# boguszjelinski/taxidispatcher

Measured on AMD Instinct MI355X. Metric: NxN assignments/sec, higher is better.
Workload: dtype int32; 1 GPU; g1 N=16384: device cost write (4N^2 B) + exact assignment, total checked == optimum; n=16384, parallelism=single GPU

## Files before the change

### taxidispatcher_amd/csrc/td_assign.hip

```cpp
#include <dlfcn.h>
#include <limits.h>
#include <stdlib.h>

#include <type_traits>

#include "td_common.h"

using namespace td;

namespace {

template <typename CT>
struct Tr;
template <>
struct Tr<uint8_t> {
    using PT = int32_t;
    static constexpr int E = 16;
    static constexpr uint32_t SENT = 0xFFu;
    static constexpr int64_t LIMIT = 254;
    static constexpr int32_t BIG = 1 << 28;
    static constexpr int32_t KMAX = INT32_MAX;
};
template <>
struct Tr<uint16_t> {
// ... 124 lines not shown
int g_sapx_min = 8;
int g_sapx_rows = 24;
int g_sap512 = 1;
int g_psap_worth = 4;
int g_bid0 = 1;
int g_defer_const = 1;
int g_shape = 1;
int g_shape_max_n = 1 << 20;
int g_narrow_price = 1;
long long g_np_plimit = NP_PLIMIT;
int g_fuse_t = 2;
int g_fuse_spec = 1;
int g_fused_rounds = 8;
int g_fuse_gen = 1;
int g_tick_rounds = 5;
int g_forest = 1;
int g_forest_min_n = 2048;
long long g_forest_w0 = 16;
long long g_forest_wx = 16;
int g_blocks = -1;
int g_blocks_min_n = 12288;
int g_zs_rounds = 4;
int g_hop_passes = 2;
int g_hop_max_rows = HOP_FMAX;
int g_lazy_cc = 1;
int g_hop_global = 1;
int g_one_trip = 1;
int g_zs_global_rounds = 6;
int g_core = 1;
int g_core_k = 64;
int g_core_min_n = 8192;
int g_core_mode = 1;
double g_core_eps = 1.0;
int g_rand_test = 1;
int g_rand_div = 8192;
int g_rand_rounds = 48;
double g_rand_corr = 0.12;
int g_core_patience = 6;
int g_solver_eps = 0;
int g_eps_theta = 8;
long long g_eps0_mult = 4;
void read_tunables()
{
    static bool done = false;
    if (done) return;
    done = true;
// ... 45 lines not shown
    if (const char *e = getenv("TD_SHAPE_MAX_N")) g_shape_max_n = atoi(e);
    if (const char *e = getenv("TD_WIDE_U16_N")) g_wide_u16_n = std::max(0, atoi(e));
    if (const char *e = getenv("TD_U16_REDO_FREE")) g_u16_redo_free = std::max(0, atoi(e));
    if (const char *e = getenv("TD_WARM_TIE_DIV")) g_warm_tie_div = std::max(1, atoi(e));
    if (const char *e = getenv("TD_LINE")) g_line = atoi(e) != 0;
    if (const char *e = getenv("TD_LINE_MIN_N")) g_line_min_n = std::max(2, atoi(e));
    if (const char *e = getenv("TD_PSAP8_GRID")) g_psap8_grid = std::max(1, std::min(192, atoi(e)));
    if (const char *e = getenv("TD_CORE")) g_core = atoi(e) != 0;
    if (const char *e = getenv("TD_CORE_K")) g_core_k = std::max(2, std::min(200, atoi(e)));
    if (const char *e = getenv("TD_CORE_MIN_N")) g_core_min_n = std::max(256, atoi(e));
    if (const char *e = getenv("TD_CORE_MODE")) g_core_mode = atoi(e);
    if (const char *e = getenv("TD_CORE_EPS")) g_core_eps = atof(e);
    if (const char *e = getenv("TD_CORE_PATIENCE")) g_core_patience = std::max(1, atoi(e));
    if (const char *e = getenv("TD_RAND_TEST")) g_rand_test = atoi(e) != 0;
    if (const char *e = getenv("TD_RAND_DIV")) g_rand_div = std::max(1, atoi(e));
    if (const char *e = getenv("TD_RAND_ROUNDS")) g_rand_rounds = std::max(1, std::min(48, atoi(e)));
    if (const char *e = getenv("TD_RAND_CORR")) g_rand_corr = atof(e);
    if (const char *e = getenv("TD_BLOCKS")) g_blocks = std::max(-1, std::min(HOP_BMAX, atoi(e)));
    if (const char *e = getenv("TD_BLOCKS_MIN_N")) g_blocks_min_n = std::max(0, atoi(e));
    if (const char *e = getenv("TD_ZS_ROUNDS")) g_zs_rounds = std::max(0, std::min(32, atoi(e)));
    if (const char *e = getenv("TD_HOP_PASSES")) g_hop_passes = std::max(0, std::min(8, atoi(e)));
    if (const char *e = getenv("TD_HOP_MAX_ROWS")) g_hop_max_rows = std::max(1, atoi(e));
    if (const char *e = getenv("TD_HOP_GLOBAL")) g_hop_global = atoi(e) != 0;
    if (const char *e = getenv("TD_ONE_TRIP")) g_one_trip = atoi(e) != 0;
    if (const char *e = getenv("TD_LAZY_CC")) g_lazy_cc = atoi(e) != 0;
    if (const char *e = getenv("TD_ZS_GLOBAL_ROUNDS")) g_zs_global_rounds = std::max(1, std::min(48, atoi(e)));
}

template <typename CT>
__device__ __forceinline__ void unpack(const uint4 &v, uint32_t *out);
template <>
__device__ __forceinline__ void unpack<uint8_t>(const uint4 &v, uint32_t *o)
{
    const uint32_t w[4] = {v.x, v.y, v.z, v.w};
#pragma unroll
    for (int k = 0; k < 4; k++) {
        o[4 * k + 0] = w[k] & 0xFFu;
        o[4 * k + 1] = (w[k] >> 8) & 0xFFu;
        o[4 * k + 2] = (w[k] >> 16) & 0xFFu;
        o[4 * k + 3] = w[k] >> 24;
    }
}
template <>
__device__ __forceinline__ void unpack<u8e>(const uint4 &v, uint32_t *o)
{
    const uint32_t w[4] = {v.x, v.y, v.z, v.w};
// ... 735 lines not shown
    for (int o = 1; o < 64; o <<= 1) {
        const int va = __shfl_up(ia, o), vb = __shfl_up(ib, o);
        if (lane >= o) ia += va, ib += vb;
    }
    if (lane == 63) s_fl2_w[0][w] = ia, s_fl2_w[1][w] = ib;
    __syncthreads();
    int basea = 0, baseb = 0;
    for (int k = 0; k < w; k++) basea += s_fl2_w[0][k], baseb += s_fl2_w[1][k];
    if (tid == T - 1) s_fl2_tot[0] = basea + ia, s_fl2_tot[1] = baseb + ib;
    free_list_fill(na, a, lista, wanta, cnta, basea + ia - cnta);
    free_list_fill(nb, b, listb, wantb, cntb, baseb + ib - cntb);
    __syncthreads();
    tota = s_fl2_tot[0], totb = s_fl2_tot[1];
}

__global__ __launch_bounds__(1024) void k_freelist(int n, const int *__restrict__ r2c, int *__restrict__ list,
                                                   int *__restrict__ ctl)
{
    if (ctl[CTL_FLAG]) return;
    const int cnt = build_free_list(n, r2c, list);
    if (threadIdx.x == 0) ctl[CTL_NFREE] = cnt;
}

#include "td_blocks.h"
#include "td_core_warm.h"

__device__ __forceinline__ void place_const_tail(int n, int *__restrict__ r2c, int *__restrict__ owner,
                                                 int *__restrict__ lista, int *__restrict__ listb,
                                                 int *__restrict__ ctl)
{
    if (ctl[CTL_NCONST] == 0) return;
    const int nr = build_free_list(n, r2c, lista, -2);
    if (nr == 0) return;
    const int nc = build_free_list(n, owner, listb, -1);
    if (nc != nr) {
        if (threadIdx.x == 0) atomicOr(&ctl[CTL_ERR], 8);
        return;
    }
    for (int k = threadIdx.x; k < nr; k += blockDim.x) {
        const int r = lista[k], j = listb[k];
        r2c[r] = j;
        owner[j] = r;
    }
}

__global__ __launch_bounds__(1024) void k_place_const(int n, int *__restrict__ r2c, int *__restrict__ owner,
                                                      int *__restrict__ lista, int *__restrict__ listb,
                                                      int *__restrict__ ctl, const int *__restrict__ gate_left = nullptr)
{
    const int flag = __hip_atomic_load(&ctl[CTL_FLAG], __ATOMIC_RELAXED, __HIP_MEMORY_SCOPE_AGENT);
    const int nconst = __hip_atomic_load(&ctl[CTL_NCONST], __ATOMIC_RELAXED, __HIP_MEMORY_SCOPE_AGENT);
    const int left = gate_left ? *gate_left : 0;
    asm volatile("" :: "v"(flag), "v"(nconst), "s"(left));
    if (flag || left != 0 || nconst == 0) return;
    place_const_tail(n, r2c, owner, lista, listb, ctl);
}

__device__ __forceinline__ void shape_decide(int n, int *__restrict__ ctl)
{
    int *sh = ctl + CTL_SHAPE;
    __threadfence();
    const int ncol = atomicAdd(&sh[0], 0);
    const int nrow = atomicAdd(&ctl[CTL_NCONST], 0);
    sh[1] = nrow;
    const int margin = n / 256 > 32 ? n / 256 : 32;
    if (ncol >= 16 && ncol - nrow >= margin) {
        sh[3] = 1;
// ... 1967 lines not shown
    *fits = h[CTL_FLAG] == 0 && *range <= (int64_t)Tr<uint32_t>::LIMIT && *range >= 0;
    sv.nconst = h[CTL_NCONST];
    if (*fits) {
        sv.nchunks = nchunks;
        sv.npad = npad;
    }
    return TD_OK;
}

int sv_complete_cc(Solver &sv)
{
    if (!sv.cc_partial) return TD_OK;
    Ctx &c = ctx();
    ProfScope ps(TD_K_COMPRESS);
    k_compress_rest<<<std::max(1, std::min(sv.nrows, c.n_cu * 8)), 256, 0, c.stream>>>(sv.n, sv.nrows, sv.row0, sv.nchunks, sv.cc_rpb, sv.d_cost,
                                                                                      (uint8_t *)sv.cc.p, (const int32_t *)sv.rowmin.p,
                                                                                      (const int *)sv.misc.p);
    TD_HIP(hipGetLastError());
    sv.cc_partial = false;
    return TD_OK;
}

template <typename CT>
int sv_hop_t(Solver &sv, int rpb, int ncols_blk, int col_lo, int nb, bool window_zero, uint8_t *ob, bool raw = false, bool gate = false)
{
    Ctx &c = ctx();
    using PT = typename Tr<CT>::PT;
    int rc;
    if ((rc = ensure(sv.hop, sizeof(HopCtl)))) return rc;
    if ((rc = ensure(sv.hoptab, sizeof(int) * (size_t)nb * HOP_FMAX * HOP_FMAX))) return rc;
    HopCtl *hc = (HopCtl *)sv.hop.p;
    int *frl = (int *)sv.list.p, *fcl = (int *)sv.pred.p;
    const int *ctl = (const int *)sv.misc.p;
    if (gate && nb != 1) return fail(TD_EINTERNAL, "a gated two-hop pass takes one block");
    const int nseg = raw && window_zero ? (ncols_blk / 4 + 1023) / 1024 : 1;
    k_hop_lists<<<nb, 1024, 0, c.stream>>>(rpb, ncols_blk, col_lo, (const int *)sv.r2c.p, (const int *)sv.owner.p, frl, fcl, hc, ctl,
                                           gate ? g_hop_max_rows : 0, nseg > 1 ? (int *)sv.hoptab.p : nullptr);
    if (raw) {
        if (!sv.d_cost || sv.n % 4) return fail(TD_EINVAL, "two-hop pass on the int32 matrix: no matrix, or n %% 4 != 0");
        if (nseg > 1)
            k_hop_table<CT, true, true><<<nb * HOP_FMAX * nseg, 256, 0, c.stream>>>(
                sv.n, sv.nrows, sv.row0, sv.n / 4, rpb, ncols_blk, col_lo, g_hop_max_rows, 1, (const CT *)sv.d_cost, (const PT *)sv.price.p,
                (const int *)sv.owner.p, frl, fcl, hc, (int *)sv.hoptab.p, ctl, (const int32_t *)sv.rowmin.p, nseg);
        else
        k_hop_table<CT, true><<<nb * HOP_FMAX, 256, 0, c.stream>>>(sv.n, sv.nrows, sv.row0, sv.n / 4, rpb, ncols_blk, col_lo, g_hop_max_rows,
                                                                   window_zero ? 1 : 0, (const CT *)sv.d_cost, (const PT *)sv.price.p,
                                                                   (const int *)sv.owner.p, frl, fcl, hc, (int *)sv.hoptab.p, ctl,
                                                                   (const int32_t *)sv.rowmin.p);
    } else {
    k_hop_table<CT><<<nb * HOP_FMAX, 256, 0, c.stream>>>(sv.n, sv.nrows, sv.row0, sv.nchunks, rpb, ncols_blk, col_lo, g_hop_max_rows,
                                                         window_zero ? 1 : 0, (const CT *)sv.cc.p, (const PT *)sv.price.p,
                                                         (const int *)sv.owner.p, frl, fcl, hc, (int *)sv.hoptab.p, ctl);
    }
    const size_t match_lds = sizeof(uint32_t) * ((size_t)HOP_FMAX * HOP_FMAX + (size_t)((rpb + 31) / 32));
    if (match_lds > 150 * 1024) return fail(TD_EINVAL, "two-hop pass: a block of that many rows does not fit the LDS");
    TD_HIP(hipFuncSetAttribute((const void *)k_hop_match<PT>, hipFuncAttributeMaxDynamicSharedMemorySize, (int)match_lds));
    k_hop_match<PT><<<nb, HOP_MATCH_T, match_lds, c.stream>>>(
        sv.nrows, sv.row0, rpb, ncols_blk, col_lo, g_hop_max_rows, (PT *)sv.price.p, (int *)sv.owner.p, (int *)sv.r2c.p, ob, frl, fcl, hc,
        (const int *)sv.hoptab.p, (int *)sv.misc.p);
    TD_HIP(hipGetLastError());
    return TD_OK;
}

int sv_phase_a(Solver &sv, int hop_passes)
{
    Ctx &c = ctx();
    const int n = sv.n, nrows = sv.nrows;
    const int rpb = n / sv.zs_V, nb = nrows / rpb;
    const int col_lo = (sv.row0 / rpb) * rpb, col_hi = col_lo + nb * rpb;
    int rc;
    if ((rc = ensure(sv.ob, (size_t)sv.npad + 64))) return rc;
    if (!sv.ob_clear) TD_HIP(hipMemsetAsync(sv.ob.p, 0, (size_t)sv.npad, c.stream));
    sv.ob_clear = false;
    ProfScope ps(TD_K_BID);
    int *ctl = (int *)sv.misc.p;
    const int ga = (col_hi - col_lo + 255) / 256;
    unsigned long long *bid = (unsigned long long *)sv.bid.p;
    auto assign = [&]() {
        k_zs_assign<<<ga, 256, 0, c.stream>>>(col_lo, col_hi, nrows, sv.row0, bid, (int32_t *)sv.price.p, (int *)sv.owner.p, (int *)sv.r2c.p,
                                              (uint8_t *)sv.ob.p, ctl);
    };
    assign();
    for (int r = 1; r <= g_zs_rounds; r++) {
        k_zs_bid<<<(nrows + 3) / 4, 256, 0, c.stream>>>(nrows, sv.row0, sv.nchunks, rpb, (const uint8_t *)sv.cc.p,
                                                                     (const uint8_t *)sv.ob.p, (const int *)sv.r2c.p, bid, ctl, r, g_tie_evict);
        assign();
    }
    TD_HIP(hipGetLastError());
    for (int p = 0; p < hop_passes; p++)
        if ((rc = sv_hop_t<uint8_t>(sv, rpb, rpb, col_lo, nb, true, (uint8_t *)sv.ob.p))) return rc;
    if (getenv("TD_DEBUG") && hop_passes > 0) {
        HopCtl h;
        TD_HIP(hipMemcpyAsync(&h, sv.hop.p, sizeof(h), hipMemcpyDeviceToHost, c.stream));
        TD_HIP(hipStreamSynchronize(c.stream));
        fprintf(stderr, "[td] phase A: %d blocks of %d rows, %d local rounds; free rows / columns per block before the last two-hop pass:", nb, rpb, g_zs_rounds);
        for (int b = 0; b < nb; b++) fprintf(stderr, " %d/%d", h.nfr[b], h.nfc[b]);
        fprintf(stderr, " | matched %d, left %d\n", h.matched, h.left);
    }
    sv.zs_done = false;
    sv.bid0_done = false;
    sv.state_ready = true;
    return TD_OK;
}

template <typename CT>
int sv_begin_t(Solver &sv)
{
    Ctx &c = ctx();
    using PT = typename Tr<CT>::PT;
    const PT padkey = (PT)(Tr<CT>::BIG << 1) | (PT)1;
    k_init_state<PT><<<(std::max(sv.npad, (int)CTL_WORDS) + 255) / 256, 256, 0, c.stream>>>(
        sv.n, sv.npad, sv.nrows, (PT *)sv.price.p, padkey, (int *)sv.owner.p, (int *)sv.r2c.p,
        (unsigned long long *)sv.bid.p, (int *)sv.misc.p, sv.defer_const ? (const int *)sv.rconst.p : nullptr, sv.probe, 0, nullptr,
// ... 525 lines not shown
        fprintf(stderr, " | parallel-sap %d | serial-sap rows %d steps %d | finisher_path 0x%llx\n", hctl[CTL_PACC], hctl[CTL_NFREE], hctl[CTL_STEPS],
                (unsigned long long)c.stats[13]);
    }
    c.stats[0] = rounds;
    c.stats[1] = 0;
    c.stats[2] = hctl[CTL_NFREE];
    c.stats[3] = hctl[CTL_STEPS];
    c.stats[4] = sv.bpc == 5 ? 4 : (sv.bpc == 6 ? 1 : sv.bpc);
    c.stats[5] = hctl[CTL_PACC];
    c.stats[10] = hctl[CTL_FOREST];
    return TD_OK;
}

int sv_readback(Solver &sv, int64_t *total, int64_t *dual, int max_rounds, int *range_flag = nullptr)
{
    Ctx &c = ctx();
    char *pin = (char *)c.pinned;
    static_assert(CTL_ALL * sizeof(int) <= FIN_OFF, "the totals sit at byte FIN_OFF of the control block");
    TD_HIP(hipMemcpyAsync(pin, sv.misc.p, FIN_OFF + 16, hipMemcpyDeviceToHost, c.stream));
    TD_HIP(hipStreamSynchronize(c.stream));
    return sv_readback_parse(sv, pin, total, dual, max_rounds, range_flag);
}

int sv_end_gated(Solver &sv, bool want_dual, int *r2c_out)
{
    Ctx &c = ctx();
    const int n = sv.n, nrows = sv.nrows;
    const int *left = (const int *)((char *)sv.hop.p + offsetof(HopCtl, left));
    int *ctl = (int *)sv.misc.p;
    unsigned long long *out = (unsigned long long *)((char *)sv.misc.p + FIN_OFF);
    int rc;
    if (want_dual && (rc = sv_complete_cc(sv))) return rc;
    ProfScope ps(TD_K_FINAL);
    if (sv.defer_const)
        k_place_const<<<1, 1024, 0, c.stream>>>(n, (int *)sv.r2c.p, (int *)sv.owner.p, (int *)sv.list.p, (int *)sv.pred.p, ctl, left);
    if (want_dual)
        k_dual<uint8_t><<<std::max(1, std::min((nrows + 3) / 4, c.n_cu * 8)), 256, 0, c.stream>>>(
            n, nrows, sv.row0, sv.nchunks, (const uint8_t *)sv.cc.p, (const int32_t *)sv.price.p, (const int32_t *)sv.rowmin.p, out, left, ctl);
    int *rec = (int *)((char *)c.pinned + REC_OFF);
    rec[REC_LEFT / sizeof(int)] = -1;
    k_final<false><<<std::min((nrows + 255) / 256, 256), 256, 0, c.stream>>>(n, nrows, sv.row0, sv.d_cost, (const int *)sv.r2c.p,
                                                                          (const int *)sv.owner.p, out, ctl, 0, CellSrc(), left, r2c_out,
                                                                          (unsigned int *)((char *)sv.misc.p + FIN_TICKET), rec);
    TD_HIP(hipGetLastError());
    return TD_OK;
}

}

namespace {

struct AssignHint {
    bool valid = false;
    int const_cols = 0, const_rows = 0, fill = 0;
    bool tick = false;
    bool gen = false;
    CellSrc src;
// ... 287 lines not shown
    int rc;
    const int keep = g_warm_bits;
    g_warm_bits = bits;
    if (cl.bpc == 2) rc = sv_warm_t<uint16_t>(sv, cl.known_range, &cl.warm_rounds, &cl.random_like);
    else if (cl.bpc == 5) rc = sv_warm_t<u32n>(sv, cl.known_range, &cl.warm_rounds, &cl.random_like);
    else rc = sv_warm_t<uint32_t>(sv, cl.known_range, &cl.warm_rounds, &cl.random_like);
    g_warm_bits = keep;
    return rc;
}

int read_left(Solver &sv, int *pin)
{
    Ctx &c = ctx();
    TD_HIP(hipMemcpyAsync(pin, (char *)sv.hop.p + offsetof(HopCtl, left), sizeof(int), hipMemcpyDeviceToHost, c.stream));
    TD_HIP(hipMemcpyAsync(pin + 1, (int *)sv.misc.p + CTL_FLAG, sizeof(int), hipMemcpyDeviceToHost, c.stream));
    TD_HIP(hipStreamSynchronize(c.stream));
    return TD_OK;
}

int block_one_trip(Solver &sv, Call &cl, Next &next)
{
    const int n = cl.n;
    int rc;
    if (g_hop_global && (rc = sv_hop_t<uint8_t>(sv, n, n, 0, 1, true, nullptr, sv.cc_partial, true))) return rc;
    const bool dev_out = is_device_ptr(cl.row_to_col);
    cl.r2c_in_pinned = !dev_out && (size_t)R2C_PIN_OFF + sizeof(int32_t) * (size_t)n <= cl.c.pinned_cap;
    int *r2c_out = dev_out ? cl.row_to_col : (cl.r2c_in_pinned ? (int *)((char *)cl.c.pinned + R2C_PIN_OFF) : nullptr);
    if ((rc = sv_end_gated(sv, cl.dual_bound != nullptr, r2c_out))) return rc;
    TD_HIP(hipStreamSynchronize(cl.c.stream));
    const char *rec = (const char *)cl.c.pinned + REC_OFF;
    const int left = ((const int *)rec)[REC_LEFT / sizeof(int)], rflag = ((const int *)rec)[CTL_FLAG];
    if (left < 0) return fail(TD_EINTERNAL, "the end-of-solve record was not written");
    if (getenv("TD_DEBUG")) fprintf(stderr, "[td] one trip: %d rows free after the two-hop passes, flag %d\n", left, rflag);
    if (left == 0 && rflag == 0) {
        int flag = 0;
        if ((rc = sv_readback_parse(sv, rec, &cl.tot, &cl.dual, cl.max_rounds, &flag))) return rc;
        cl.c.stats[1] = 0;
        cl.c.stats[6] = 0;
        cl.r2c_on_device = dev_out;
        return go(next, Next::solved);
    }
    cl.r2c_in_pinned = false;
    cl.round_cap = std::min(cl.max_rounds, g_zs_global_rounds);
    return TD_OK;
}

int block_read_back(Solver &sv, Call &cl)
{
    const int n = cl.n;
    int rc;
    int *pin = (int *)cl.c.pinned;
// ... 908 lines not shown
```

### taxidispatcher_amd/csrc/td_blocks.h

```cpp


struct HopCtl {
    int nfr[HOP_BMAX], nfc[HOP_BMAX];
    int left;
    int matched;
    int pad[2];
};

__device__ __forceinline__ uint32_t zs_zero_bytes(uint32_t w)
{
    return ~(((w & 0x7F7F7F7Fu) + 0x7F7F7F7Fu) | w | 0x7F7F7F7Fu);
}


__global__ __launch_bounds__(256) void k_zs_bid(int nrows, int row0, int nchunks, int rpb, const uint8_t *__restrict__ cc,
                                                const uint8_t *__restrict__ ob, const int *__restrict__ r2c,
                                                unsigned long long *__restrict__ bid, const int *__restrict__ ctl, int round,
                                                int tie_evict)
{
    const int lane = threadIdx.x & 63;
    const int lrow = blockIdx.x * 4 + __builtin_amdgcn_readfirstlane(threadIdx.x >> 6);
    const int flag = ctl[CTL_FLAG], col = r2c[min(lrow, nrows - 1)];
    asm volatile("" :: "s"(flag), "s"(col));
    if (flag || lrow >= nrows || col != -1) return;
// ... 80 lines not shown
            if (threadIdx.x == 0) hc->nfr[lb] = 0, hc->nfc[lb] = 0;
            return;
        }
    }
    const int *rs = r2c + (size_t)lb * rpb, *os = owner + col_lo + (size_t)lb * ncols_blk;
    int cntr, cntc;
    if (rpb == ncols_blk) free_list_count2(rpb, rs, -1, os, -1, cntr, cntc);
    else cntr = free_list_count(rpb, rs, -1), cntc = free_list_count(ncols_blk, os, -1);
    asm volatile("" :: "v"(cntr), "v"(cntc));
    if (flag) return;
    int nfr, nfc;
    build_free_list2(rpb, rs, frl + (size_t)lb * rpb, -1, cntr, ncols_blk, os, fcl + (size_t)lb * ncols_blk, -1, cntc, nfr, nfc);
    if (threadIdx.x == 0) {
        hc->nfr[lb] = nfr;
        hc->nfc[lb] = nfc;
        if (lb == 0) hc->left = 0, hc->matched = 0;
    }
    if (tab_preset) {
        int4 *t4 = reinterpret_cast<int4 *>(tab_preset + (size_t)lb * HOP_FMAX * HOP_FMAX);
        for (int k = threadIdx.x; k < min(nfr, HOP_FMAX) * (HOP_FMAX / 4); k += 1024) t4[k] = make_int4(HOP_NONE, HOP_NONE, HOP_NONE, HOP_NONE);
    }
}

template <typename CT, bool RAW = false, bool SPLIT = false>
__global__ __launch_bounds__(256) void k_hop_table(int n, int nrows, int row0, int nchunks, int rpb, int ncols_blk, int col_lo,
                                                   int max_rows, int window_zero, const CT *__restrict__ cc,
                                                   const typename Tr<CT>::PT *__restrict__ pk, const int *__restrict__ owner,
                                                   const int *__restrict__ frl, const int *__restrict__ fcl,
                                                   const HopCtl *__restrict__ hc, int *__restrict__ tab,
                                                   const int *__restrict__ ctl, const int32_t *__restrict__ rowmin = nullptr,
                                                   int nseg = 1)
{
    using PT = typename Tr<CT>::PT;
    constexpr int E = RAW ? 4 : Tr<CT>::E;
    __shared__ int s_tab[HOP_FMAX];
    constexpr int CHT = RAW ? 4 : 1;
    __shared__ int s_cand[256 * E * CHT];
    __shared__ int s_hr[256 * E * CHT], s_hj[256 * E * CHT];
    __shared__ int s_fc[HOP_FMAX];
    __shared__ int s_ncand, s_nhit;
    __shared__ long long s_v[4];
    constexpr int HU = 4;
    const int seg = SPLIT ? (int)blockIdx.x % nseg : 0, ba = SPLIT ? (int)blockIdx.x / nseg : (int)blockIdx.x;
    const int lb = ba / HOP_FMAX, a = ba % HOP_FMAX;
    const int tid = threadIdx.x, lane = tid & 63, w = tid >> 6;
    int flag = ctl[CTL_FLAG];
    int nfr = hc->nfr[lb], nfc_all = hc->nfc[lb];
    int fr_a = frl[(size_t)lb * rpb + min(a, rpb - 1)];
    int fc_t = fcl[(size_t)lb * ncols_blk + min(tid & (HOP_FMAX - 1), ncols_blk - 1)];
    asm volatile("" :: "s"(flag), "s"(nfr), "s"(nfc_all), "s"(fr_a), "v"(fc_t));
    if (flag) return;
    if (nfr > max_rows || a >= min(nfr, HOP_FMAX)) return;
    const int lrow = lb * rpb + fr_a;
    const size_t pitch = (size_t)nchunks * E;
    const unsigned char *rp = reinterpret_cast<const unsigned char *>(cc) + (size_t)lrow * pitch * (RAW ? 4 : sizeof(CT));
    const int32_t mn = RAW ? rowmin[lrow] : 0;
    auto cells = [&](const uint4 &raw, uint32_t *c) {
        if constexpr (RAW) {
            c[0] = (uint32_t)((int32_t)raw.x - mn), c[1] = (uint32_t)((int32_t)raw.y - mn);
            c[2] = (uint32_t)((int32_t)raw.z - mn), c[3] = (uint32_t)((int32_t)raw.w - mn);
        } else
            unpack<CT>(raw, c);
    };
    auto ecell = [&](int rl, int col) -> long long {
        if constexpr (RAW) return (long long)(uint32_t)(reinterpret_cast<const int32_t *>(cc)[(size_t)rl * pitch + col] - rowmin[rl]);
        else return (long long)(uint32_t)cc[(size_t)rl * pitch + col];
    };
    const int nfc = min(nfc_all, HOP_FMAX);
    const int cb = col_lo + lb * ncols_blk;
    if (tid < nfc) s_fc[tid] = fc_t;
    int *tab_row = tab + ((size_t)lb * HOP_FMAX + a) * HOP_FMAX;
    if (!SPLIT && tid < HOP_FMAX) s_tab[tid] = INT_MAX;
    if (tid == 0) s_ncand = 0, s_nhit = 0;
    const int ch_lo = window_zero ? (col_lo + lb * ncols_blk) / E : 0;
    const int ch_n = window_zero ? (ncols_blk + E - 1) / E : nchunks;
    long long v = 0;
    if (!window_zero) {
        long long mv = LLONG_MAX;
        for (int t = tid; t < ch_n; t += 256) {
            uint32_t c[E];
            cells(*reinterpret_cast<const uint4 *>(rp + (size_t)(ch_lo + t) * 16), c);
            PT pv[E];
            const int j0 = (ch_lo + t) * E;
            if constexpr (sizeof(PT) == 4) {
                const int4 *pp = reinterpret_cast<const int4 *>(pk + j0);
#pragma unroll
                for (int q = 0; q < E / 4; q++) {
                    const int4 x = pp[q];
                    pv[4 * q + 0] = x.x, pv[4 * q + 1] = x.y, pv[4 * q + 2] = x.z, pv[4 * q + 3] = x.w;
                }
            } else {
#pragma unroll
                for (int e = 0; e < E; e++) pv[e] = pk[j0 + e];
            }
// ... 70 lines not shown
            for (int q = 0; q < HU; q++) {
                const int p = min(p0 + q * 256 + tid, np - 1);
                const int h = p / nfc, b = p - h * nfc;
                const int rl = s_hr[h], j = s_hj[h], jb = cb + s_fc[b];
                rg[q] = rl + row0, bb[q] = b;
                live[q] = SPLIT || s_tab[b] > rg[q];
                du[q] = dx[q] = 0;
                if (live[q]) {
                    du[q] = ecell(rl, j) + (long long)(pk[j] >> 1);
                    dx[q] = ecell(rl, jb) + (long long)(pk[jb] >> 1);
                }
            }
#pragma unroll
            for (int q = 0; q < HU; q++)
                if (live[q] && p0 + q * 256 + tid < np && du[q] == dx[q]) atomicMin(&dst[bb[q]], rg[q]);
        }
        __syncthreads();
        if (tid == 0) s_ncand = 0, s_nhit = 0;
        __syncthreads();
    }
    if (!SPLIT && tid < HOP_FMAX) tab_row[tid] = s_tab[tid] == INT_MAX ? -1 : s_tab[tid];
}

constexpr int HOP_MATCH_T = 256;
template <typename PT>
__global__ __launch_bounds__(HOP_MATCH_T) void k_hop_match(int nrows, int row0, int rpb, int ncols_blk, int col_lo, int max_rows,
                                                           PT *__restrict__ pk, int *__restrict__ owner, int *__restrict__ r2c,
                                                           uint8_t *__restrict__ ob, const int *__restrict__ frl,
                                                           const int *__restrict__ fcl, HopCtl *__restrict__ hc,
                                                           const int *__restrict__ tab, int *__restrict__ ctl)
{
    extern __shared__ uint32_t s_hop_dyn[];
    __shared__ int s_st[HOP_FMAX];
    __shared__ int s_win[HOP_FMAX][2];
    constexpr int HOP_TAB_U = 4;
    const int lb = blockIdx.x;
    const int tid = threadIdx.x;
    const int *fr = frl + (size_t)lb * rpb, *fc = fcl + (size_t)lb * ncols_blk;
    const int4 *src = reinterpret_cast<const int4 *>(tab + (size_t)lb * HOP_FMAX * HOP_FMAX);
    int flag = ctl[CTL_FLAG];
    int nfr = hc->nfr[lb], nfc_all = hc->nfc[lb];
    int fr_t = fr[min(tid & (HOP_FMAX - 1), rpb - 1)];
    int4 x0[HOP_TAB_U];
#pragma unroll
    for (int q = 0; q < HOP_TAB_U; q++) x0[q] = src[tid + q * HOP_MATCH_T];
    asm volatile("" :: "s"(flag), "s"(nfr), "s"(nfc_all), "v"(fr_t), "v"(x0[0].x), "v"(x0[0].y), "v"(x0[0].z), "v"(x0[0].w),
                 "v"(x0[1].x), "v"(x0[1].y), "v"(x0[1].z), "v"(x0[1].w), "v"(x0[2].x), "v"(x0[2].y), "v"(x0[2].z), "v"(x0[2].w),
                 "v"(x0[3].x), "v"(x0[3].y), "v"(x0[3].z), "v"(x0[3].w));
    static_assert(HOP_TAB_U == 4, "the operand list above");
    if (flag) return;
    if (nfr == 0) return;
    if (nfr > max_rows) {
        if (tid == 0) atomicAdd(&hc->left, nfr);
        return;
    }
    const int na = min(nfr, HOP_FMAX), nc = min(nfc_all, HOP_FMAX);
    int *s_tab = reinterpret_cast<int *>(s_hop_dyn);
    uint32_t *s_usedr = s_hop_dyn + HOP_FMAX * HOP_FMAX;
    const int blk_row0 = row0 + lb * rpb;
    const int my_i = tid < na ? blk_row0 + fr_t : 0;
    {
        int4 *dst = reinterpret_cast<int4 *>(s_tab);
        auto norm = [&](int r, int col) { return (r == HOP_NONE || col >= nc) ? -1 : r; };
        auto stage = [&](int k, const int4 &x) {
            const int col = (k * 4) & (HOP_FMAX - 1);
            dst[k] = make_int4(norm(x.x, col), norm(x.y, col + 1), norm(x.z, col + 2), norm(x.w, col + 3));
        };
        const int nq = na * (HOP_FMAX / 4);
#pragma unroll
        for (int q = 0; q < HOP_TAB_U; q++)
            if (tid + q * HOP_MATCH_T < nq) stage(tid + q * HOP_MATCH_T, x0[q]);
        for (int k0 = tid + HOP_TAB_U * HOP_MATCH_T; k0 < nq; k0 += HOP_TAB_U * HOP_MATCH_T) {
            int4 x[HOP_TAB_U];
#pragma unroll
            for (int q = 0; q < HOP_TAB_U; q++) x[q] = src[min(k0 + q * HOP_MATCH_T, nq - 1)];
#pragma unroll
            for (int q = 0; q < HOP_TAB_U; q++)
                if (k0 + q * HOP_MATCH_T < nq) stage(k0 + q * HOP_MATCH_T, x[q]);
        }
        for (int k = tid; k < (rpb + 31) / 32; k += HOP_MATCH_T) s_usedr[k] = 0u;
        if (tid < na) {
            const uint32_t hsh = ((uint32_t)my_i + 1u) * 0x9E3779B1u;
            s_st[tid] = nc ? (int)(((uint64_t)(hsh ^ (hsh >> 15)) * (uint64_t)nc) >> 32) : 0;
        }
    }
    __syncthreads();
    if (tid < 64) {
        const int lane = tid;
        auto entry = [&](int a, int col) -> int {
            const int r = s_tab[min(a, HOP_FMAX - 1) * HOP_FMAX + col];
            return a < na ? r : -1;
        };
        auto used = [&](int r) -> bool {
            const int rb = max(r - blk_row0, 0);
            const uint32_t word = s_usedr[rb >> 5];
            return r < 0 || ((word >> (rb & 31)) & 1u);
        };
        unsigned long long usedc0 = 0ull, usedc1 = 0ull;
        int done = 0, r_prev = -1;
        int ra0 = entry(0, lane), ra1 = entry(0, lane + 64);
        int rb0 = entry(1, lane), rb1 = entry(1, lane + 64);
        bool ua0 = used(ra0), ua1 = used(ra1);
        int st = s_st[0];
        for (int a = 0; a < na; a++) {
            const int rc0 = entry(a + 2, lane), rc1 = entry(a + 2, lane + 64);
            const bool ub0 = used(rb0), ub1 = used(rb1);
            const int st_nx = s_st[min(a + 1, HOP_FMAX - 1)];
            const unsigned long long m0 = __ballot(!ua0 && ra0 != r_prev) & ~usedc0;
            const unsigned long long m1 = __ballot(!ua1 && ra1 != r_prev) & ~usedc1;
            int rw = -1, cw = 0;
            if (m0 | m1) {
                const unsigned long long h0 = st < 64 ? m0 & (~0ull << st) : 0ull;
                const unsigned long long h1 = st < 64 ? m1 : m1 & (~0ull << (st - 64));
                if (h0 | h1) cw = h0 ? __builtin_ctzll(h0) : 64 + __builtin_ctzll(h1);
                else cw = m0 ? __builtin_ctzll(m0) : 64 + __builtin_ctzll(m1);
                rw = __builtin_amdgcn_readlane(cw < 64 ? ra0 : ra1, cw & 63);
                if (cw < 64) usedc0 |= 1ull << cw;
                else usedc1 |= 1ull << (cw - 64);
                r_prev = rw;
                done++;
            }
            if (lane == 0) {
                s_win[a][0] = rw, s_win[a][1] = cw;
                if (rw >= 0) {
                    const int rb = rw - blk_row0;
                    atomicOr(&s_usedr[rb >> 5], 1u << (rb & 31));
                }
            }
            __builtin_amdgcn_fence(__ATOMIC_ACQ_REL, "wavefront");
            ra0 = rb0, ra1 = rb1, ua0 = ub0, ua1 = ub1;
            rb0 = rc0, rb1 = rc1;
            st = st_nx;
        }
        if (lane == 0) {
            atomicAdd(&hc->left, nfr - done);
            atomicAdd(&hc->matched, done);
        }
    }
    __syncthreads();
    if (tid < na && s_win[tid][0] >= 0) {
        const int r = s_win[tid][0], i_g = my_i;
        const int rl = r - row0, il = i_g - row0;
        const int j = r2c[rl], jp = col_lo + lb * ncols_blk + fc[s_win[tid][1]];
        r2c[il] = j;
        owner[j] = i_g;
        r2c[rl] = jp;
        owner[jp] = r;
        pk[jp] = pk[jp] | (PT)1;
        if (ob) ob[jp] = 1;
    }
}
```

Baseline: 31.07 million assignments/s.

## Run extra two-hop passes inside k_hop_match and fold constant-row placement

The repeated two-hop passes are folded into a single k_hop_match launch. After each pass the kernel rebuilds the free-row and free-column lists, recomputes the hop table in LDS and loops again. When the pass covers the whole matrix, the same kernel also places the deferred constant rows, so the separate k_place_const launch is dropped. This removes several kernel launches and the list/table kernels between passes. In exchange, one 256-thread block per row-block now serially recomputes the table rows, and the kernel uses more LDS.

Result: no change. 31.30 million assignments/s, median of 6 (+0.7%).

```diff
diff --git a/taxidispatcher_amd/csrc/td_assign.hip b/taxidispatcher_amd/csrc/td_assign.hip
--- a/taxidispatcher_amd/csrc/td_assign.hip
+++ b/taxidispatcher_amd/csrc/td_assign.hip
@@ -170,6 +170,7 @@
 int g_blocks_min_n = 12288;
 int g_zs_rounds = 4;
 int g_hop_passes = 2;
+int g_hop_inblock = 1;
 int g_hop_max_rows = HOP_FMAX;
 int g_lazy_cc = 1;
 int g_hop_global = 1;
@@ -261,6 +262,7 @@
     if (const char *e = getenv("TD_HOP_PASSES")) g_hop_passes = std::max(0, std::min(8, atoi(e)));
     if (const char *e = getenv("TD_HOP_MAX_ROWS")) g_hop_max_rows = std::max(1, atoi(e));
     if (const char *e = getenv("TD_HOP_GLOBAL")) g_hop_global = atoi(e) != 0;
+    if (const char *e = getenv("TD_HOP_INBLOCK")) g_hop_inblock = atoi(e) != 0;
     if (const char *e = getenv("TD_ONE_TRIP")) g_one_trip = atoi(e) != 0;
     if (const char *e = getenv("TD_LAZY_CC")) g_lazy_cc = atoi(e) != 0;
     if (const char *e = getenv("TD_ZS_GLOBAL_ROUNDS")) g_zs_global_rounds = std::max(1, std::min(48, atoi(e)));
@@ -1042,9 +1044,6 @@
     if (threadIdx.x == 0) ctl[CTL_NFREE] = cnt;
 }
 
-#include "td_blocks.h"
-#include "td_core_warm.h"
-
 __device__ __forceinline__ void place_const_tail(int n, int *__restrict__ r2c, int *__restrict__ owner,
                                                  int *__restrict__ lista, int *__restrict__ listb,
                                                  int *__restrict__ ctl)
@@ -1063,6 +1062,9 @@
         owner[j] = r;
     }
 }
+
+#include "td_blocks.h"
+#include "td_core_warm.h"
 
 __global__ __launch_bounds__(1024) void k_place_const(int n, int *__restrict__ r2c, int *__restrict__ owner,
                                                       int *__restrict__ lista, int *__restrict__ listb,
@@ -3076,7 +3078,8 @@
 }
 
 template <typename CT>
-int sv_hop_t(Solver &sv, int rpb, int ncols_blk, int col_lo, int nb, bool window_zero, uint8_t *ob, bool raw = false, bool gate = false)
+int sv_hop_t(Solver &sv, int rpb, int ncols_blk, int col_lo, int nb, bool window_zero, uint8_t *ob, bool raw = false, bool gate = false,
+             int extra_passes = 0, bool place_const = false)
 {
     Ctx &c = ctx();
     using PT = typename Tr<CT>::PT;
@@ -3087,6 +3090,10 @@
     int *frl = (int *)sv.list.p, *fcl = (int *)sv.pred.p;
     const int *ctl = (const int *)sv.misc.p;
     if (gate && nb != 1) return fail(TD_EINTERNAL, "a gated two-hop pass takes one block");
+    if (extra_passes && (!window_zero || raw || !std::is_same<CT, uint8_t>::value))
+        return fail(TD_EINTERNAL, "two-hop passes inside k_hop_match: in-block passes on the 1-byte narrow copy only");
+    if (place_const && (nb != 1 || rpb != sv.n || sv.nrows != sv.n || sv.row0 != 0))
+        return fail(TD_EINTERNAL, "the constant rows are placed by a two-hop pass over the whole matrix only");
     const int nseg = raw && window_zero ? (ncols_blk / 4 + 1023) / 1024 : 1;
     k_hop_lists<<<nb, 1024, 0, c.stream>>>(rpb, ncols_blk, col_lo, (const int *)sv.r2c.p, (const int *)sv.owner.p, frl, fcl, hc, ctl,
                                            gate ? g_hop_max_rows : 0, nseg > 1 ? (int *)sv.hoptab.p : nullptr);
@@ -3107,11 +3114,18 @@
                                                          (const int *)sv.owner.p, frl, fcl, hc, (int *)sv.hoptab.p, ctl);
     }
     const size_t match_lds = sizeof(uint32_t) * ((size_t)HOP_FMAX * HOP_FMAX + (size_t)((rpb + 31) / 32));
-    if (match_lds > 150 * 1024) return fail(TD_EINVAL, "two-hop pass: a block of that many rows does not fit the LDS");
+    static size_t match_static = 0;
+    if (!match_static) {
+        hipFuncAttributes fa;
+        TD_HIP(hipFuncGetAttributes(&fa, (const void *)k_hop_match<PT>));
+        match_static = fa.sharedSizeBytes;
+    }
+    if (match_lds + match_static > 160 * 1024)
+        return fail(TD_EINVAL, "two-hop pass: a block of that many rows does not fit the LDS");
     TD_HIP(hipFuncSetAttribute((const void *)k_hop_match<PT>, hipFuncAttributeMaxDynamicSharedMemorySize, (int)match_lds));
     k_hop_match<PT><<<nb, HOP_MATCH_T, match_lds, c.stream>>>(
-        sv.nrows, sv.row0, rpb, ncols_blk, col_lo, g_hop_max_rows, (PT *)sv.price.p, (int *)sv.owner.p, (int *)sv.r2c.p, ob, frl, fcl, hc,
-        (const int *)sv.hoptab.p, (int *)sv.misc.p);
+        sv.n, sv.nrows, sv.row0, sv.nchunks, rpb, ncols_blk, col_lo, g_hop_max_rows, (const uint8_t *)sv.cc.p, (PT *)sv.price.p,
+        (int *)sv.owner.p, (int *)sv.r2c.p, ob, frl, fcl, hc, (const int *)sv.hoptab.p, (int *)sv.misc.p, extra_passes, place_const ? 1 : 0);
     TD_HIP(hipGetLastError());
     return TD_OK;
 }
@@ -3141,8 +3155,11 @@
         assign();
     }
     TD_HIP(hipGetLastError());
-    for (int p = 0; p < hop_passes; p++)
-        if ((rc = sv_hop_t<uint8_t>(sv, rpb, rpb, col_lo, nb, true, (uint8_t *)sv.ob.p))) return rc;
+    if (g_hop_inblock) {
+        if (hop_passes > 0 && (rc = sv_hop_t<uint8_t>(sv, rpb, rpb, col_lo, nb, true, (uint8_t *)sv.ob.p, false, false, hop_passes - 1))) return rc;
+    } else
+        for (int p = 0; p < hop_passes; p++)
+            if ((rc = sv_hop_t<uint8_t>(sv, rpb, rpb, col_lo, nb, true, (uint8_t *)sv.ob.p))) return rc;
     if (getenv("TD_DEBUG") && hop_passes > 0) {
         HopCtl h;
         TD_HIP(hipMemcpyAsync(&h, sv.hop.p, sizeof(h), hipMemcpyDeviceToHost, c.stream));
@@ -3714,7 +3731,7 @@
     return sv_readback_parse(sv, pin, total, dual, max_rounds, range_flag);
 }
 
-int sv_end_gated(Solver &sv, bool want_dual, int *r2c_out)
+int sv_end_gated(Solver &sv, bool want_dual, int *r2c_out, bool const_placed)
 {
     Ctx &c = ctx();
     const int n = sv.n, nrows = sv.nrows;
@@ -3724,7 +3741,7 @@
     int rc;
     if (want_dual && (rc = sv_complete_cc(sv))) return rc;
     ProfScope ps(TD_K_FINAL);
-    if (sv.defer_const)
+    if (sv.defer_const && !const_placed)
         k_place_const<<<1, 1024, 0, c.stream>>>(n, (int *)sv.r2c.p, (int *)sv.owner.p, (int *)sv.list.p, (int *)sv.pred.p, ctl, left);
     if (want_dual)
         k_dual<uint8_t><<<std::max(1, std::min((nrows + 3) / 4, c.n_cu * 8)), 256, 0, c.stream>>>(
@@ -4058,11 +4075,12 @@
 {
     const int n = cl.n;
     int rc;
-    if (g_hop_global && (rc = sv_hop_t<uint8_t>(sv, n, n, 0, 1, true, nullptr, sv.cc_partial, true))) return rc;
+    const bool fold_const = g_hop_inblock && g_hop_global && sv.defer_const;
+    if (g_hop_global && (rc = sv_hop_t<uint8_t>(sv, n, n, 0, 1, true, nullptr, sv.cc_partial, true, 0, fold_const))) return rc;
     const bool dev_out = is_device_ptr(cl.row_to_col);
     cl.r2c_in_pinned = !dev_out && (size_t)R2C_PIN_OFF + sizeof(int32_t) * (size_t)n <= cl.c.pinned_cap;
     int *r2c_out = dev_out ? cl.row_to_col : (cl.r2c_in_pinned ? (int *)((char *)cl.c.pinned + R2C_PIN_OFF) : nullptr);
-    if ((rc = sv_end_gated(sv, cl.dual_bound != nullptr, r2c_out))) return rc;
+    if ((rc = sv_end_gated(sv, cl.dual_bound != nullptr, r2c_out, fold_const))) return rc;
     TD_HIP(hipStreamSynchronize(cl.c.stream));
     const char *rec = (const char *)cl.c.pinned + REC_OFF;
     const int left = ((const int *)rec)[REC_LEFT / sizeof(int)], rflag = ((const int *)rec)[CTL_FLAG];
diff --git a/taxidispatcher_amd/csrc/td_blocks.h b/taxidispatcher_amd/csrc/td_blocks.h
--- a/taxidispatcher_amd/csrc/td_blocks.h
+++ b/taxidispatcher_amd/csrc/td_blocks.h
@@ -126,14 +126,10 @@
     }
 }
 
-template <typename CT, bool RAW = false, bool SPLIT = false>
-__global__ __launch_bounds__(256) void k_hop_table(int n, int nrows, int row0, int nchunks, int rpb, int ncols_blk, int col_lo,
-                                                   int max_rows, int window_zero, const CT *__restrict__ cc,
-                                                   const typename Tr<CT>::PT *__restrict__ pk, const int *__restrict__ owner,
-                                                   const int *__restrict__ frl, const int *__restrict__ fcl,
-                                                   const HopCtl *__restrict__ hc, int *__restrict__ tab,
-                                                   const int *__restrict__ ctl, const int32_t *__restrict__ rowmin = nullptr,
-                                                   int nseg = 1)
+template <typename CT, bool RAW, bool SPLIT>
+__device__ __forceinline__ void hop_table_row(int n, int nrows, int row0, int nchunks, int rpb, int ncols_blk, int col_lo, int window_zero,
+                                              const CT *cc, const typename Tr<CT>::PT *pk, const int *owner, const int32_t *rowmin,
+                                              int lb, int seg, int nfc_all, int fr_a, int fc_t, int *tab_row)
 {
     using PT = typename Tr<CT>::PT;
     constexpr int E = RAW ? 4 : Tr<CT>::E;
@@ -145,16 +141,7 @@
     __shared__ int s_ncand, s_nhit;
     __shared__ long long s_v[4];
     constexpr int HU = 4;
-    const int seg = SPLIT ? (int)blockIdx.x % nseg : 0, ba = SPLIT ? (int)blockIdx.x / nseg : (int)blockIdx.x;
-    const int lb = ba / HOP_FMAX, a = ba % HOP_FMAX;
     const int tid = threadIdx.x, lane = tid & 63, w = tid >> 6;
-    int flag = ctl[CTL_FLAG];
-    int nfr = hc->nfr[lb], nfc_all = hc->nfc[lb];
-    int fr_a = frl[(size_t)lb * rpb + min(a, rpb - 1)];
-    int fc_t = fcl[(size_t)lb * ncols_blk + min(tid & (HOP_FMAX - 1), ncols_blk - 1)];
-    asm volatile("" :: "s"(flag), "s"(nfr), "s"(nfc_all), "s"(fr_a), "v"(fc_t));
-    if (flag) return;
-    if (nfr > max_rows || a >= min(nfr, HOP_FMAX)) return;
     const int lrow = lb * rpb + fr_a;
     const size_t pitch = (size_t)nchunks * E;
     const unsigned char *rp = reinterpret_cast<const unsigned char *>(cc) + (size_t)lrow * pitch * (RAW ? 4 : sizeof(CT));
@@ -173,7 +160,6 @@
     const int nfc = min(nfc_all, HOP_FMAX);
     const int cb = col_lo + lb * ncols_blk;
     if (tid < nfc) s_fc[tid] = fc_t;
-    int *tab_row = tab + ((size_t)lb * HOP_FMAX + a) * HOP_FMAX;
     if (!SPLIT && tid < HOP_FMAX) s_tab[tid] = INT_MAX;
     if (tid == 0) s_ncand = 0, s_nhit = 0;
     const int ch_lo = window_zero ? (col_lo + lb * ncols_blk) / E : 0;
@@ -290,21 +276,53 @@
     if (!SPLIT && tid < HOP_FMAX) tab_row[tid] = s_tab[tid] == INT_MAX ? -1 : s_tab[tid];
 }
 
+template <typename CT, bool RAW = false, bool SPLIT = false>
+__global__ __launch_bounds__(256) void k_hop_table(int n, int nrows, int row0, int nchunks, int rpb, int ncols_blk, int col_lo,
+                                                   int max_rows, int window_zero, const CT *__restrict__ cc,
+                                                   const typename Tr<CT>::PT *__restrict__ pk, const int *__restrict__ owner,
+                                                   const int *__restrict__ frl, const int *__restrict__ fcl,
+                                                   const HopCtl *__restrict__ hc, int *__restrict__ tab,
+                                                   const int *__restrict__ ctl, const int32_t *__restrict__ rowmin = nullptr,
+                                                   int nseg = 1)
+{
+    const int seg = SPLIT ? (int)blockIdx.x % nseg : 0, ba = SPLIT ? (int)blockIdx.x / nseg : (int)blockIdx.x;
+    const int lb = ba / HOP_FMAX, a = ba % HOP_FMAX;
+    const int tid = threadIdx.x;
+    int flag = ctl[CTL_FLAG];
+    int nfr = hc->nfr[lb], nfc_all = hc->nfc[lb];
+    int fr_a = frl[(size_t)lb * rpb + min(a, rpb - 1)];
+    int fc_t = fcl[(size_t)lb * ncols_blk + min(tid & (HOP_FMAX - 1), ncols_blk - 1)];
+    asm volatile("" :: "s"(flag), "s"(nfr), "s"(nfc_all), "s"(fr_a), "v"(fc_t));
+    if (flag) return;
+    if (nfr > max_rows || a >= min(nfr, HOP_FMAX)) return;
+    hop_table_row<CT, RAW, SPLIT>(n, nrows, row0, nchunks, rpb, ncols_blk, col_lo, window_zero, cc, pk, owner, rowmin, lb, seg, nfc_all, fr_a,
+                                  fc_t, tab + ((size_t)lb * HOP_FMAX + a) * HOP_FMAX);
+}
+
+__device__ __forceinline__ void hop_republish()
+{
+    __builtin_amdgcn_fence(__ATOMIC_RELEASE, "agent");
+    __syncthreads();
+    __builtin_amdgcn_fence(__ATOMIC_ACQUIRE, "agent");
+}
+
 constexpr int HOP_MATCH_T = 256;
 template <typename PT>
-__global__ __launch_bounds__(HOP_MATCH_T) void k_hop_match(int nrows, int row0, int rpb, int ncols_blk, int col_lo, int max_rows,
-                                                           PT *__restrict__ pk, int *__restrict__ owner, int *__restrict__ r2c,
-                                                           uint8_t *__restrict__ ob, const int *__restrict__ frl,
-                                                           const int *__restrict__ fcl, HopCtl *__restrict__ hc,
-                                                           const int *__restrict__ tab, int *__restrict__ ctl)
+__global__ __launch_bounds__(HOP_MATCH_T) void k_hop_match(int n, int nrows, int row0, int nchunks, int rpb, int ncols_blk, int col_lo,
+                                                           int max_rows, const uint8_t *__restrict__ cc, PT *__restrict__ pk,
+                                                           int *__restrict__ owner, int *__restrict__ r2c, uint8_t *__restrict__ ob,
+                                                           int *__restrict__ frl, int *__restrict__ fcl, HopCtl *__restrict__ hc,
+                                                           const int *__restrict__ tab, int *__restrict__ ctl, int extra_passes,
+                                                           int place_const)
 {
     extern __shared__ uint32_t s_hop_dyn[];
     __shared__ int s_st[HOP_FMAX];
     __shared__ int s_win[HOP_FMAX][2];
+    __shared__ int s_done;
     constexpr int HOP_TAB_U = 4;
     const int lb = blockIdx.x;
     const int tid = threadIdx.x;
-    const int *fr = frl + (size_t)lb * rpb, *fc = fcl + (size_t)lb * ncols_blk;
+    int *fr = frl + (size_t)lb * rpb, *fc = fcl + (size_t)lb * ncols_blk;
     const int4 *src = reinterpret_cast<const int4 *>(tab + (size_t)lb * HOP_FMAX * HOP_FMAX);
     int flag = ctl[CTL_FLAG];
     int nfr = hc->nfr[lb], nfc_all = hc->nfc[lb];
@@ -312,109 +330,149 @@
     int4 x0[HOP_TAB_U];
 #pragma unroll
     for (int q = 0; q < HOP_TAB_U; q++) x0[q] = src[tid + q * HOP_MATCH_T];
+    const int left_in = __hip_atomic_load(&hc->left, __ATOMIC_RELAXED, __HIP_MEMORY_SCOPE_AGENT);
+    const int nconst = __hip_atomic_load(&ctl[CTL_NCONST], __ATOMIC_RELAXED, __HIP_MEMORY_SCOPE_AGENT);
     asm volatile("" :: "s"(flag), "s"(nfr), "s"(nfc_all), "v"(fr_t), "v"(x0[0].x), "v"(x0[0].y), "v"(x0[0].z), "v"(x0[0].w),
                  "v"(x0[1].x), "v"(x0[1].y), "v"(x0[1].z), "v"(x0[1].w), "v"(x0[2].x), "v"(x0[2].y), "v"(x0[2].z), "v"(x0[2].w),
-                 "v"(x0[3].x), "v"(x0[3].y), "v"(x0[3].z), "v"(x0[3].w));
+                 "v"(x0[3].x), "v"(x0[3].y), "v"(x0[3].z), "v"(x0[3].w), "v"(left_in), "v"(nconst));
     static_assert(HOP_TAB_U == 4, "the operand list above");
     if (flag) return;
-    if (nfr == 0) return;
-    if (nfr > max_rows) {
-        if (tid == 0) atomicAdd(&hc->left, nfr);
-        return;
-    }
-    const int na = min(nfr, HOP_FMAX), nc = min(nfc_all, HOP_FMAX);
-    int *s_tab = reinterpret_cast<int *>(s_hop_dyn);
-    uint32_t *s_usedr = s_hop_dyn + HOP_FMAX * HOP_FMAX;
-    const int blk_row0 = row0 + lb * rpb;
-    const int my_i = tid < na ? blk_row0 + fr_t : 0;
-    {
-        int4 *dst = reinterpret_cast<int4 *>(s_tab);
-        auto norm = [&](int r, int col) { return (r == HOP_NONE || col >= nc) ? -1 : r; };
-        auto stage = [&](int k, const int4 &x) {
-            const int col = (k * 4) & (HOP_FMAX - 1);
-            dst[k] = make_int4(norm(x.x, col), norm(x.y, col + 1), norm(x.z, col + 2), norm(x.w, col + 3));
-        };
-        const int nq = na * (HOP_FMAX / 4);
-#pragma unroll
-        for (int q = 0; q < HOP_TAB_U; q++)
-            if (tid + q * HOP_MATCH_T < nq) stage(tid + q * HOP_MATCH_T, x0[q]);
-        for (int k0 = tid + HOP_TAB_U * HOP_MATCH_T; k0 < nq; k0 += HOP_TAB_U * HOP_MATCH_T) {
-            int4 x[HOP_TAB_U];
-#pragma unroll
-            for (int q = 0; q < HOP_TAB_U; q++) x[q] = src[min(k0 + q * HOP_MATCH_T, nq - 1)];
-#pragma unroll
-            for (int q = 0; q < HOP_TAB_U; q++)
-                if (k0 + q * HOP_MATCH_T < nq) stage(k0 + q * HOP_MATCH_T, x[q]);
-        }
-        for (int k = tid; k < (rpb + 31) / 32; k += HOP_MATCH_T) s_usedr[k] = 0u;
-        if (tid < na) {
-            const uint32_t hsh = ((uint32_t)my_i + 1u) * 0x9E3779B1u;
-            s_st[tid] = nc ? (int)(((uint64_t)(hsh ^ (hsh >> 15)) * (uint64_t)nc) >> 32) : 0;
-        }
-    }
-    __syncthreads();
-    if (tid < 64) {
-        const int lane = tid;
-        auto entry = [&](int a, int col) -> int {
-            const int r = s_tab[min(a, HOP_FMAX - 1) * HOP_FMAX + col];
-            return a < na ? r : -1;
-        };
-        auto used = [&](int r) -> bool {
-            const int rb = max(r - blk_row0, 0);
-            const uint32_t word = s_usedr[rb >> 5];
-            return r < 0 || ((word >> (rb & 31)) & 1u);
-        };
-        unsigned long long usedc0 = 0ull, usedc1 = 0ull;
-        int done = 0, r_prev = -1;
-        int ra0 = entry(0, lane), ra1 = entry(0, lane + 64);
-        int rb0 = entry(1, lane), rb1 = entry(1, lane + 64);
-        bool ua0 = used(ra0), ua1 = used(ra1);
-        int st = s_st[0];
-        for (int a = 0; a < na; a++) {
-            const int rc0 = entry(a + 2, lane), rc1 = entry(a + 2, lane + 64);
-            const bool ub0 = used(rb0), ub1 = used(rb1);
-            const int st_nx = s_st[min(a + 1, HOP_FMAX - 1)];
-            const unsigned long long m0 = __ballot(!ua0 && ra0 != r_prev) & ~usedc0;
-            const unsigned long long m1 = __ballot(!ua1 && ra1 != r_prev) & ~usedc1;
-            int rw = -1, cw = 0;
-            if (m0 | m1) {
-                const unsigned long long h0 = st < 64 ? m0 & (~0ull << st) : 0ull;
-                const unsigned long long h1 = st < 64 ? m1 : m1 & (~0ull << (st - 64));
-                if (h0 | h1) cw = h0 ? __builtin_ctzll(h0) : 64 + __builtin_ctzll(h1);
-                else cw = m0 ? __builtin_ctzll(m0) : 64 + __builtin_ctzll(m1);
-                rw = __builtin_amdgcn_readlane(cw < 64 ? ra0 : ra1, cw & 63);
-                if (cw < 64) usedc0 |= 1ull << cw;
-                else usedc1 |= 1ull << (cw - 64);
-                r_prev = rw;
-                done++;
-            }
-            if (lane == 0) {
-                s_win[a][0] = rw, s_win[a][1] = cw;
-                if (rw >= 0) {
-                    const int rb = rw - blk_row0;
-                    atomicOr(&s_usedr[rb >> 5], 1u << (rb & 31));
-                }
-            }
-            __builtin_amdgcn_fence(__ATOMIC_ACQ_REL, "wavefront");
-            ra0 = rb0, ra1 = rb1, ua0 = ub0, ua1 = ub1;
-            rb0 = rc0, rb1 = rc1;
-            st = st_nx;
-        }
-        if (lane == 0) {
-            atomicAdd(&hc->left, nfr - done);
-            atomicAdd(&hc->matched, done);
-        }
-    }
-    __syncthreads();
-    if (tid < na && s_win[tid][0] >= 0) {
-        const int r = s_win[tid][0], i_g = my_i;
-        const int rl = r - row0, il = i_g - row0;
-        const int j = r2c[rl], jp = col_lo + lb * ncols_blk + fc[s_win[tid][1]];
-        r2c[il] = j;
-        owner[j] = i_g;
-        r2c[rl] = jp;
-        owner[jp] = r;
-        pk[jp] = pk[jp] | (PT)1;
-        if (ob) ob[jp] = 1;
-    }
-}
+    int left_out = left_in;
+    if (nfr == 0 || nfr > max_rows) {
+        if (nfr && tid == 0) atomicAdd(&hc->left, nfr);
+        if (!place_const) return;
+        if (nfr) left_out = nfr;
+    } else {
+        int *s_tab = reinterpret_cast<int *>(s_hop_dyn);
+        uint32_t *s_usedr = s_hop_dyn + HOP_FMAX * HOP_FMAX;
+        const int blk_row0 = row0 + lb * rpb;
+        for (int pass = 0;; pass++) {
+            const int na = min(nfr, HOP_FMAX), nc = min(nfc_all, HOP_FMAX);
+            const int my_i = tid < na ? blk_row0 + fr_t : 0;
+            if (pass == 0) {
+                int4 *dst = reinterpret_cast<int4 *>(s_tab);
+                auto norm = [&](int r, int col) { return (r == HOP_NONE || col >= nc) ? -1 : r; };
+                auto stage = [&](int k, const int4 &x) {
+                    const int col = (k * 4) & (HOP_FMAX - 1);
+                    dst[k] = make_int4(norm(x.x, col), norm(x.y, col + 1), norm(x.z, col + 2), norm(x.w, col + 3));
+                };
+                const int nq = na * (HOP_FMAX / 4);
+#pragma unroll
+                for (int q = 0; q < HOP_TAB_U; q++)
+                    if (tid + q * HOP_MATCH_T < nq) stage(tid + q * HOP_MATCH_T, x0[q]);
+                for (int k0 = tid + HOP_TAB_U * HOP_MATCH_T; k0 < nq; k0 += HOP_TAB_U * HOP_MATCH_T) {
+                    int4 x[HOP_TAB_U];
+#pragma unroll
+                    for (int q = 0; q < HOP_TAB_U; q++) x[q] = src[min(k0 + q * HOP_MATCH_T, nq - 1)];
+#pragma unroll
+                    for (int q = 0; q < HOP_TAB_U; q++)
+                        if (k0 + q * HOP_MATCH_T < nq) stage(k0 + q * HOP_MATCH_T, x[q]);
+                }
+            }
+            for (int k = tid; k < (rpb + 31) / 32; k += HOP_MATCH_T) s_usedr[k] = 0u;
+            if (tid < na) {
+                const uint32_t hsh = ((uint32_t)my_i + 1u) * 0x9E3779B1u;
+                s_st[tid] = nc ? (int)(((uint64_t)(hsh ^ (hsh >> 15)) * (uint64_t)nc) >> 32) : 0;
+            }
+            __syncthreads();
+            if (tid < 64) {
+                const int lane = tid;
+                auto entry = [&](int a, int col) -> int {
+                    const int r = s_tab[min(a, HOP_FMAX - 1) * HOP_FMAX + col];
+                    return a < na ? r : -1;
+                };
+                auto used = [&](int r) -> bool {
+                    const int rb = max(r - blk_row0, 0);
+                    const uint32_t word = s_usedr[rb >> 5];
+                    return r < 0 || ((word >> (rb & 31)) & 1u);
+                };
+                unsigned long long usedc0 = 0ull, usedc1 = 0ull;
+                int done = 0, r_prev = -1;
+                int ra0 = entry(0, lane), ra1 = entry(0, lane + 64);
+                int rb0 = entry(1, lane), rb1 = entry(1, lane + 64);
+                bool ua0 = used(ra0), ua1 = used(ra1);
+                int st = s_st[0];
+                for (int a = 0; a < na; a++) {
+                    const int rc0 = entry(a + 2, lane), rc1 = entry(a + 2, lane + 64);
+                    const bool ub0 = used(rb0), ub1 = used(rb1);
+                    const int st_nx = s_st[min(a + 1, HOP_FMAX - 1)];
+                    const unsigned long long m0 = __ballot(!ua0 && ra0 != r_prev) & ~usedc0;
+                    const unsigned long long m1 = __ballot(!ua1 && ra1 != r_prev) & ~usedc1;
+                    int rw = -1, cw = 0;
+                    if (m0 | m1) {
+                        const unsigned long long h0 = st < 64 ? m0 & (~0ull << st) : 0ull;
+                        const unsigned long long h1 = st < 64 ? m1 : m1 & (~0ull << (st - 64));
+                        if (h0 | h1) cw = h0 ? __builtin_ctzll(h0) : 64 + __builtin_ctzll(h1);
+                        else cw = m0 ? __builtin_ctzll(m0) : 64 + __builtin_ctzll(m1);
+                        rw = __builtin_amdgcn_readlane(cw < 64 ? ra0 : ra1, cw & 63);
+                        if (cw < 64) usedc0 |= 1ull << cw;
+                        else usedc1 |= 1ull << (cw - 64);
+                        r_prev = rw;
+                        done++;
+                    }
+                    if (lane == 0) {
+                        s_win[a][0] = rw, s_win[a][1] = cw;
+                        if (rw >= 0) {
+                            const int rb = rw - blk_row0;
+                            atomicOr(&s_usedr[rb >> 5], 1u << (rb & 31));
+                        }
+                    }
+                    __builtin_amdgcn_fence(__ATOMIC_ACQ_REL, "wavefront");
+                    ra0 = rb0, ra1 = rb1, ua0 = ub0, ua1 = ub1;
+                    rb0 = rc0, rb1 = rc1;
+                    st = st_nx;
+                }
+                if (lane == 0) s_done = done;
+            }
+            __syncthreads();
+            if (tid < na && s_win[tid][0] >= 0) {
+                const int r = s_win[tid][0], i_g = my_i;
+                const int rl = r - row0, il = i_g - row0;
+                const int j = r2c[rl], jp = col_lo + lb * ncols_blk + fc[s_win[tid][1]];
+                r2c[il] = j;
+                owner[j] = i_g;
+                r2c[rl] = jp;
+                owner[jp] = r;
+                pk[jp] = pk[jp] | (PT)1;
+                if (ob) ob[jp] = 1;
+            }
+            const int done = s_done;
+            if (pass >= extra_passes || done == 0) {
+                if (tid == 0) {
+                    atomicAdd(&hc->left, nfr - done);
+                    atomicAdd(&hc->matched, done);
+                }
+                left_out = nfr - done;
+                break;
+            }
+            hop_republish();
+            const int *rs = r2c + (size_t)lb * rpb, *os = owner + col_lo + (size_t)lb * ncols_blk;
+            int cntr, cntc;
+            if (rpb == ncols_blk) free_list_count2(rpb, rs, -1, os, -1, cntr, cntc);
+            else cntr = free_list_count(rpb, rs, -1), cntc = free_list_count(ncols_blk, os, -1);
+            build_free_list2(rpb, rs, fr, -1, cntr, ncols_blk, os, fc, -1, cntc, nfr, nfc_all);
+            if (tid == 0) hc->nfr[lb] = nfr, hc->nfc[lb] = nfc_all;
+            if (nfr == 0) {
+                left_out = 0;
+                break;
+            }
+            if (nfr > max_rows) {
+                if (tid == 0) atomicAdd(&hc->left, nfr);
+                left_out = nfr;
+                break;
+            }
+            hop_republish();
+            fr_t = fr[min(tid & (HOP_FMAX - 1), rpb - 1)];
+            if constexpr (std::is_same<PT, typename Tr<uint8_t>::PT>::value) {
+                const int fc_t = fc[min(tid & (HOP_FMAX - 1), ncols_blk - 1)];
+                for (int a = 0; a < min(nfr, HOP_FMAX); a++)
+                    hop_table_row<uint8_t, false, false>(n, nrows, row0, nchunks, rpb, ncols_blk, col_lo, 1, cc, pk, owner, nullptr, lb, 0, nfc_all,
+                                                         fr[a], fc_t, s_tab + a * HOP_FMAX);
+            }
+        }
+    }
+    if (place_const && left_out == 0 && nconst != 0) {
+        hop_republish();
+        place_const_tail(n, r2c, owner, frl, fcl, ctl);
+    }
+}
```
